# yzang2019/tendermint-fork

Measured on AMD Instinct MI355X. Metric: ed25519 verifies/sec at 1/8 MI355X, higher is better.
Workload: dtype u32 (GF(2^255-19) radix 2^25.5 limbs, int64 accumulate); 1 GPU; C2: raw batch of 1048576 ed25519 signatures per GPU; signatures_per_gpu=1048576, key_cache=False, parallelism=shard-per-gpu x1

## Files before the change

include/tmed25519.h:

```cpp
#ifndef TMED25519_H
#define TMED25519_H

#include <stddef.h>
#include <stdint.h>

#ifdef __cplusplus
extern "C" {
#endif

#define TMED_OK 0
#define TMED_EINVAL (-1)
#define TMED_ENODEV (-2)
#define TMED_EHIP (-3)
#define TMED_ENOMEM (-4)
#define TMED_ENOKEYSET (-5)
#define TMED_EINTERNAL (-6)

typedef struct tmed_ctx tmed_ctx;

int tmed_device_count(void);

int tmed_init(int device, tmed_ctx **out);
void tmed_destroy(tmed_ctx *ctx);
const char *tmed_strerror(int code);
// ... 50 lines not shown
int tmed_verify_batch_keyset_zip215_device(tmed_ctx *ctx, uint64_t handle, const uint32_t *d_val_idx,
                                           const uint8_t *d_sigs, const uint8_t *d_msgs, const uint32_t *d_msg_off,
                                           size_t n, uint8_t *d_out_valid, void *stream);

#define TMED_RULE_GO 0
#define TMED_RULE_ZIP215 1
int tmed_set_rule(tmed_ctx *ctx, int rule);
int tmed_rule(const tmed_ctx *ctx);


typedef struct {
  const char *chain_id;
  uint32_t chain_id_len;
  int64_t height;
  int32_t round;
  const uint8_t *block_hash;
  uint32_t block_hash_len;
  uint32_t psh_total;
  const uint8_t *psh_hash;
  uint32_t psh_hash_len;
} tmed_vote_template;

int tmed_vote_sign_bytes(const tmed_vote_template *t, size_t n, const uint8_t *flags, const int64_t *ts_seconds,
                         const int32_t *ts_nanos, uint8_t *out, size_t out_cap, uint32_t *out_off, size_t *out_len);


int tmed_valu_peak(tmed_ctx *ctx, int kind, double *giga_ops_per_s);

void tmed_test_pool_jitter(int max_us);
void tmed_test_stream_delay(int us);

int tmed_test_joint_rows(tmed_ctx *ctx, const uint8_t *a, const uint8_t *r, const uint8_t *dneg, size_t n,
                         uint8_t *rows);

int tmed_test_b_table_entry(tmed_ctx *ctx, int table, uint32_t window, uint32_t j, int32_t out[30]);
int tmed_test_table_chain(tmed_ctx *ctx, int table, uint64_t handle, int radix_bits, uint32_t corrupt_window,
                          uint32_t corrupt_j, uint64_t *rows, uint64_t *n_bad, uint64_t first_bad[16]);

int tmed_test_zip_msm(tmed_ctx *ctx, uint32_t n, const uint8_t *points, const int16_t *digits, const uint8_t *c,
                      uint32_t lo, uint32_t cnt, int32_t windows[640], uint32_t ctot[8], uint32_t *flag);

int tmed_test_key_order(tmed_ctx *ctx, const uint32_t *val_idx, uint32_t n, uint32_t nkeys, uint32_t index_base,
                        uint32_t *perm_out, uint32_t *cursor_out, uint32_t *nbins_out, uint32_t *shift_out);
int tmed_test_finish(tmed_ctx *ctx, uint32_t m, const int32_t *xyz, const uint8_t *r, const uint32_t *perm,
                     uint32_t fin_base, const uint8_t *bits_in, uint8_t *bits_out);
int tmed_test_finish_zip215(tmed_ctx *ctx, uint32_t m, const int32_t *xyz, const uint8_t *r, const uint32_t *perm,
                            uint32_t fin_base, const uint8_t *bits_in, uint8_t *bits_out);

int tmed_debug_zero_bits(void *out, size_t cap, size_t *n);


typedef struct {
  const uint8_t *hash;
  uint32_t hash_len;
  uint32_t psh_total;
  const uint8_t *psh_hash;
  uint32_t psh_hash_len;
} tmed_block_id;

typedef struct {
  size_t n;
  const uint8_t *pubkeys;
  const int64_t *powers;
  const uint8_t *addresses;
  int64_t total_power;
  uint64_t keyset;
// ... 331 lines not shown
```

tendermint-fork_amd/csrc/kernels.h:

```cpp
#pragma once
#include <hip/hip_runtime.h>
#include <stddef.h>
#include <stdint.h>

#include "ge25519.h"
#include "signbytes.h"

namespace tmed {

struct KernelTimer {
  static constexpr int kMax = 160;
  hipEvent_t ev[kMax];
  int kind[kMax];
  int n = 0;
  void mark(hipStream_t s, int k) {
    if (n < kMax) { kind[n] = k; (void)hipEventRecord(ev[n++], s); }
  }
};

constexpr uint32_t kThreadsPerBlock = 256;
constexpr uint32_t kSlabSlotBytes = 8 * 128;
constexpr uint32_t kSlabJointSlotBytes = 12 * 128;
inline size_t slab_bytes(uint32_t slots) { return (size_t)slots * kSlabJointSlotBytes; }

// ... 63 lines not shown
                             hipStream_t stream);
hipError_t launch_comb_fill(const int32_t *bases, uint32_t n, int4 *comb, hipStream_t stream);
#ifndef TMED_COMBA_BITS
#define TMED_COMBA_BITS 12
#endif
constexpr int kCombABits = TMED_COMBA_BITS;
constexpr int kCombAWindows = 253 / kCombABits;
constexpr int kCombATopField = 253 - kCombABits * (kCombAWindows - 1);
constexpr uint32_t kCombAEntries = (1u << (kCombABits - 1)) + 1;
constexpr uint32_t kCombATopMax = (1u << (kCombATopField - 1)) + 1;
constexpr uint32_t kCombATopGroups = (kCombATopMax + 127) / 128;
constexpr uint32_t kCombATopEntries = kCombATopGroups * 128 + 1;
static_assert(kCombABits >= 10 && kCombABits <= 12 && kCombATopField >= kCombABits, "comb radix");
constexpr size_t kCombARowsPerKey = (size_t)(kCombAWindows - 1) * kCombAEntries + kCombATopEntries;
constexpr size_t kCombABytesPerKey = kCombARowsPerKey * kCombEntryInt4 * 16;
constexpr size_t comba_row(int w, uint32_t j) { return (size_t)w * kCombAEntries + j; }
hipError_t launch_build_comba(const uint8_t *pubs, uint32_t n, int32_t *bases, int4 *comba, hipStream_t stream);
hipError_t launch_verify_keyset(const uint32_t *val_idx, uint32_t nkeys, const uint8_t *key_pub, const uint8_t *key_ok,
                                const int4 *const *acomb, const int4 *bcomb, const uint8_t *sig, const uint8_t *msgs,
                                const uint32_t *off, uint32_t n, uint8_t *out, int4 *prep, uint32_t stride,
                                int4 *fin, int4 *fin_pre, hipStream_t stream, bool msg_slots = false,
                                KernelTimer *timer = nullptr, uint32_t *perm = nullptr,
                                uint32_t *order_scratch = nullptr, const int4 *bcomb24 = nullptr,
                                const int4 *const *acomba = nullptr, int rule = kRuleGo);
constexpr uint32_t kKeyOrderMaxKeys = 1u << 24;
uint32_t key_order_scratch_words(uint32_t n, uint32_t nkeys);
uint32_t key_order_shift(uint32_t nkeys);
hipError_t launch_key_order(const uint32_t *val_idx, uint32_t n, uint32_t nkeys, uint32_t *scratch, uint32_t *perm,
                            uint32_t index_base, hipStream_t stream);

hipError_t launch_test_delay(hipStream_t stream, uint32_t us);
hipError_t launch_test_joint_rows(const uint8_t *a, const uint8_t *r, const uint8_t *dneg, uint32_t n, int4 *rows,
                                  hipStream_t stream);
struct ChainPlan {
  const int4 *base;
  const int4 *const *chunks;
  const uint8_t *ok;
  uint64_t units, rows_per_unit;
  uint32_t windows, entries, top_entries, top_chain_last, step_bits;
};
hipError_t launch_table_chain(const ChainPlan &p, uint64_t *d_out, hipStream_t stream);
hipError_t launch_table_corrupt(int4 *row, hipStream_t stream);
hipError_t launch_window_stats(const int4 *prep, uint32_t stride, uint32_t count, uint32_t *d_hist,
                               hipStream_t stream);

constexpr uint32_t kLatMax = 1u << 16;
struct VoteAsm;
hipError_t launch_verify_keyset_lat(const uint32_t *val_idx, uint32_t nkeys, const uint8_t *key_pub, const uint8_t *key_ok,
                                    const int4 *const *acomb, const int4 *bcomb, const uint8_t *sig, const uint8_t *msgs,
                                    const uint32_t *off, uint32_t n, uint8_t *out, int4 *fin, int4 *dec,
                                    hipStream_t stream, bool msg_slots = false, const VoteAsm *va = nullptr,
                                    int rule = kRuleGo);

constexpr uint32_t kGLatMax = 1u << 16;
constexpr size_t kGLatHandBytes = (size_t)kGLatMax * (6 * 2 + 7) * 16;
struct VoteAsm {
  const uint8_t *tmpl;
  const uint32_t *tmpl_idx;
  const uint8_t *flags;
  const int64_t *ts_sec;
  const int32_t *ts_nanos;
};

hipError_t launch_verify_glat(const uint8_t *pub, const uint8_t *sig, const uint8_t *msgs, const uint32_t *off,
                              uint32_t n, uint8_t *out, const int4 *comb16, int4 *hand, hipStream_t stream,
                              bool msg_slots = false, KernelTimer *timer = nullptr, const VoteAsm *va = nullptr);
// ... 21 lines not shown
```

tendermint-fork_amd/csrc/kernels.hip:

```cpp
#include "kernels.h"
#include "verify_core.h"
#include "verify_hs.h"
#include "kernel_util.h"
#include "rows.h"
#include "votes_dev.h"

namespace tmed {

__device__ int4 kIdentityRow[8] = {{1, 0, 0, 0}, {0, 0, 0, 0}, {1, 0, 0, 0}, {0, 0, 0, 0},
                                          {1, 0, 0, 0}, {0, 0, 0, 0}, {0, 0, 0, 0}, {0, 0, 0, 0}};

__device__ __forceinline__ void slab_st(int4 *p, int4 v) { *p = v; }
__device__ __forceinline__ int4 slab_ld(const int4 *p) { return *p; }

template <int ROWS>
struct SlabTabN {
  int4 *base;
  uint32_t slot;

  __device__ __forceinline__ const int4 *row(int j) const {
    return j == 0 ? kIdentityRow : base + ((size_t)slot * ROWS + (j - 1)) * 8;
  }

  __device__ __forceinline__ void store(int j, const ge_cached &c) const {
    if (j == 0) return;
    int4 *r = base + ((size_t)slot * ROWS + (j - 1)) * 8;
    const fe *fs[4] = {&c.YpX, &c.YmX, &c.Z, &c.T2d};
#pragma unroll
    for (int f = 0; f < 4; f++) {
      uint32_t w[8];
      fe_pack256(w, *fs[f]);
      slab_st(r + 2 * f, make_int4((int)w[0], (int)w[1], (int)w[2], (int)w[3]));
      slab_st(r + 2 * f + 1, make_int4((int)w[4], (int)w[5], (int)w[6], (int)w[7]));
    }
  }
  int4 pv[8];
  __device__ __forceinline__ void prefetch(int j, bool swap = false) {
    const int4 *r = row(j);
    const int sx = swap ? 2 : 0;
#pragma unroll
    for (int q = 0; q < 8; q++) pv[q] = slab_ld(r + (q < 4 ? (q ^ sx) : q));
  }
  __device__ __forceinline__ void take(ge_cached &c) const {
    fe *fs[4] = {&c.YpX, &c.YmX, &c.Z, &c.T2d};
#pragma unroll
    for (int f = 0; f < 4; f++) {
      const uint32_t w[8] = {(uint32_t)pv[2 * f].x, (uint32_t)pv[2 * f].y, (uint32_t)pv[2 * f].z,
                             (uint32_t)pv[2 * f].w, (uint32_t)pv[2 * f + 1].x, (uint32_t)pv[2 * f + 1].y,
                             (uint32_t)pv[2 * f + 1].z, (uint32_t)pv[2 * f + 1].w};
      fe_unpack256(*fs[f], w);
    }
  }
};
using SlabTab = SlabTabN<8>;
using SlabTabJ = SlabTabN<kJointRows>;
static_assert(kSlabSlotBytes == 8 * 128 && kSlabJointSlotBytes == kJointRows * 128, "slab rows are 128 B");

typedef __attribute__((address_space(1))) void global_void;
typedef __attribute__((address_space(3))) void lds_void;

template <int BITS>
struct BPf {
  static constexpr int kBits = BITS;
  const int4 *tab;
  int4 *buf;
  uint32_t lane;
  __device__ __forceinline__ void prefetch(int j) const {
    __builtin_amdgcn_s_waitcnt(0xc07f);
#pragma unroll
    for (int q = 0; q < 8; q++)
      __builtin_amdgcn_global_load_lds((global_void *)(tab + (size_t)j * 8 + q), (lds_void *)(buf + q * 64), 16, 0, 0);
  }
  __device__ __forceinline__ void take(ge_niels &e) const { niels_load(e, buf + lane, 64); }
};

constexpr uint32_t kHsBlock = kThreadsPerBlock;

constexpr int kPrepWaves = 3;
__global__ __launch_bounds__(kHsBlock, kPrepWaves) void verify_prep_kernel(
    const uint8_t *__restrict__ pub, const uint8_t *__restrict__ sig, MsgSrc ms, uint32_t base, uint32_t count,
    int4 *__restrict__ prep, uint32_t stride, uint32_t *__restrict__ place) {
  const uint32_t slot = blockIdx.x * blockDim.x + threadIdx.x;
  if (place && slot == 0) place[0] = place[1] = 0;
  if (slot >= count) return;
  const uint32_t i = base + slot;
  uint32_t pw[8];
  bool sok;
  {
    uint32_t sw[16], k[8], h[16];
// ... 107 lines not shown
  for (int j = 0; j < 8; j++) { w[j] = (int32_t)cr[j]; w[13 + j] = (int32_t)er[j]; }
#pragma unroll
  for (int j = 0; j < 5; j++) w[8 + j] = (int32_t)dr[j];
#pragma unroll
  for (int j = 0; j < 10; j++) { w[21 + j] = Rx.v[j]; w[31 + j] = Ry.v[j]; }
  w[41] = ((ok && rok) ? 1 : 0) | (dneg ? 2 : 0) | (W << 8);
  w[42] = (int32_t)slot;
  w[43] = 0;
#pragma unroll
  for (int q = 4; q < 9; q++) {
    const int4 v = prep[(size_t)q * stride + slot];
    w[28 + 4 * q] = v.x; w[29 + 4 * q] = v.y; w[30 + 4 * q] = v.z; w[31 + 4 * q] = v.w;
  }
  const bool front = W > kHsWSmall;
  const uint64_t act = __ballot(1), sm = __ballot(front);
  const uint32_t lane = threadIdx.x & 63u;
  const uint64_t below = lane ? (~0ull >> (64 - lane)) : 0ull;
  uint32_t fs = 0, fl = 0;
  if (lane == (uint32_t)__builtin_ctzll(act)) {
    const uint32_t ns = (uint32_t)__builtin_popcountll(sm), nl = (uint32_t)__builtin_popcountll(act & ~sm);
    if (ns) fs = atomicAdd(&place[0], ns);
    if (nl) fl = atomicAdd(&place[1], nl);
  }
  const int leader = __builtin_ctzll(act);
  fs = (uint32_t)__shfl((int)fs, leader);
  fl = (uint32_t)__shfl((int)fl, leader);
  const uint32_t pos = front ? fs + (uint32_t)__builtin_popcountll(sm & below)
                             : count - 1u - (fl + (uint32_t)__builtin_popcountll(act & ~sm & below));
#pragma unroll
  for (int q = 0; q < kPrepHsInt4; q++)
    prep2[(size_t)q * stride + pos] = make_int4(w[4 * q], w[4 * q + 1], w[4 * q + 2], w[4 * q + 3]);
}

struct HsDigitsDev {
  const int4 *p2;
  uint32_t stride, slot;
  bool active;
  __device__ __forceinline__ uint32_t word(int w) const {
    return active ? reinterpret_cast<const uint32_t *>(p2 + (size_t)(w >> 2) * stride + slot)[w & 3] : 0x88888888u;
  }
  __device__ __forceinline__ uint32_t cword(int w) const { return word(w); }
  __device__ __forceinline__ uint32_t dword(int w) const { return w < 5 ? word(8 + w) : 0x88888888u; }
};

constexpr int kHsWaves = 2;
template <int BB>
__global__ __launch_bounds__(kHsBlock, kHsWaves) void verify_main_hs_kernel(
    uint32_t base, uint32_t count, const int4 *__restrict__ prep, const int4 *__restrict__ prep2, uint32_t stride,
    int4 *__restrict__ slab, const int4 *__restrict__ btab, uint8_t *__restrict__ out, int zip215) {
  __shared__ int4 sbl[kHsBlock / 64][8 * 64];
  __shared__ int4 sbh[kHsBlock / 64][8 * 64];
  const uint32_t slot = blockIdx.x * blockDim.x + threadIdx.x;
  const bool active = slot < count;
  int32_t w[64];
#pragma unroll
  for (int q = 3; q < kPrepHsInt4; q++) {
    const int4 v = active ? prep2[(size_t)q * stride + slot] : make_int4(0, 0, 0, 0);
    w[4 * q] = v.x; w[4 * q + 1] = v.y; w[4 * q + 2] = v.z; w[4 * q + 3] = v.w;
  }
  uint32_t er[8];
#pragma unroll
  for (int j = 0; j < 8; j++) er[j] = (uint32_t)w[13 + j];
  if (BB == 16) {
    uint32_t e[8];
#pragma unroll
    for (int j = 0; j < 8; j++) e[j] = er[j];
    sc_recode_b<16>(er, e);
  }
  fe Rx, Ry;
#pragma unroll
  for (int j = 0; j < 10; j++) { Rx.v[j] = w[21 + j]; Ry.v[j] = w[31 + j]; }
  ge_p3 A;
#pragma unroll
  for (int j = 0; j < 10; j++) { A.X.v[j] = w[44 + j]; A.Y.v[j] = w[54 + j]; }
  if (!active) { fe_1(A.Y); fe_1(Ry); }
  fe_1(A.Z);
  fe_mul(A.T, A.X, A.Y);
  const int flags = w[41];
  int W = active ? (flags >> 8) : 29;
#pragma unroll
  for (int o = 32; o > 0; o >>= 1) {
    const int x = __shfl_xor(W, o);
    W = x > W ? x : W;
  }
  W = __builtin_amdgcn_readfirstlane(W);
  if (W < 29) W = 29;
  if (W > 64) W = 64;
  const uint32_t lane = threadIdx.x & 63u, wv = threadIdx.x >> 6;
  const HsDigitsDev ds{prep2, stride, slot, active};
  SlabTabJ tj{slab, slot};
  const size_t hi = BB == 26 ? (size_t)kB26Entries * kCombEntryInt4 : (size_t)8 * kB16Entries * kCombEntryInt4;
  BPf<BB> bl{btab, sbl[wv], lane};
  BPf<BB> bh{btab + hi, sbh[wv], lane};
  const bool id = verify_main_hsj(ds, (flags & 2) != 0, er, W, A, Rx, Ry, tj, bl, bh, zip215 != 0);
  if (active) out[base + (uint32_t)w[42]] = ((flags & 1) && id) ? 1 : 0;
}

__global__ __launch_bounds__(kThreadsPerBlock) void window_stats_kernel(const int4 *__restrict__ prep2, uint32_t stride,
                                                                       uint32_t count, uint32_t *__restrict__ lane_hist,
                                                                       uint32_t *__restrict__ wave_hist) {
  __shared__ uint32_t lh[65], wh[65];
  for (uint32_t b = threadIdx.x; b < 65; b += blockDim.x) lh[b] = wh[b] = 0;
  __syncthreads();
  const uint32_t slot = blockIdx.x * blockDim.x + threadIdx.x;
  const bool active = slot < count;
  int W = active ? (prep2[(size_t)10 * stride + slot].y >> 8) : 0;
  if (W < 0 || W > 64) W = 64;
  if (active) atomicAdd(&lh[W], 1u);
  int m = W;
#pragma unroll
  for (int o = 32; o > 0; o >>= 1) {
    const int x = __shfl_xor(m, o);
    m = x > m ? x : m;
  }
  if ((threadIdx.x & 63u) == 0 && slot < count) atomicAdd(&wh[m], 1u);
  __syncthreads();
  for (uint32_t b = threadIdx.x; b < 65; b += blockDim.x) {
    if (lh[b]) atomicAdd(&lane_hist[b], lh[b]);
    if (wh[b]) atomicAdd(&wave_hist[b], wh[b]);
  }
}

__global__ __launch_bounds__(kHsBlock) void test_joint_rows_kernel(const uint8_t *__restrict__ a,
                                                                   const uint8_t *__restrict__ r,
                                                                   const uint8_t *__restrict__ dneg, uint32_t n,
                                                                   int4 *__restrict__ rows) {
  const uint32_t i = blockIdx.x * blockDim.x + threadIdx.x;
  if (i >= n) return;
  uint32_t aw[8], rw[8];
  load_row_words(aw, a + 32 * (size_t)i, 2);
  load_row_words(rw, r + 32 * (size_t)i, 2);
  ge_p3 A, R, P, Q;
  ge_frombytes_go(A, aw);
  ge_frombytes_go(R, rw);
  hs_points(P, Q, dneg[i] != 0, A, R.X, R.Y);
  SlabTabJ tj{rows, i};
  build_table_joint(tj, P, Q);
}

hipError_t launch_test_joint_rows(const uint8_t *a, const uint8_t *r, const uint8_t *dneg, uint32_t n, int4 *rows,
                                  hipStream_t stream) {
  if (n == 0) return hipSuccess;
  hipLaunchKernelGGL(test_joint_rows_kernel, dim3((n + kHsBlock - 1) / kHsBlock), dim3(kHsBlock), 0, stream, a, r,
                     dneg, n, rows);
  return hipGetLastError();
}

__global__ __launch_bounds__(64) void test_delay_kernel(uint32_t iters) {
  for (uint32_t i = 0; i < iters; i++) __builtin_amdgcn_s_sleep(127);
}

hipError_t launch_test_delay(hipStream_t stream, uint32_t us) {
  if (us == 0) return hipSuccess;
  hipLaunchKernelGGL(test_delay_kernel, dim3(1), dim3(64), 0, stream, (us < 100000u ? us : 100000u) / 3u + 1u);
  return hipGetLastError();
}

hipError_t launch_window_stats(const int4 *prep, uint32_t stride, uint32_t count, uint32_t *d_hist,
                               hipStream_t stream) {
  if (count == 0) return hipSuccess;
  hipError_t e = hipMemsetAsync(d_hist, 0, 2 * 65 * sizeof(uint32_t), stream);
  if (e != hipSuccess) return e;
  hipLaunchKernelGGL(window_stats_kernel, dim3((count + kThreadsPerBlock - 1) / kThreadsPerBlock),
                     dim3(kThreadsPerBlock), 0, stream, prep + (size_t)kPrepInt4 * stride, stride, count, d_hist,
                     d_hist + 65);
  return hipGetLastError();
}

struct FinDev {
  const int4 *fin;
  int4 *pre;
  const uint8_t *sig;
  uint8_t *out;
  uint32_t fin_base, lane, L, m;
  const uint32_t *perm;
  __device__ __forceinline__ int count() const { return lane < m ? (int)((m - lane + L - 1) / L) : 0; }
  __device__ __forceinline__ uint32_t slot(int j) const { return lane + (uint32_t)j * L; }
// ... 722 lines not shown
```

tendermint-fork_amd/csrc/tmed_capi.hip:

```cpp
#include <hip/hip_runtime.h>
#include <stdlib.h>
#include <string.h>

#include <algorithm>
#include <map>
#include <mutex>
#include <new>
#include <string>

#include "../../include/tmed25519.h"
#include "kernels.h"

#include "call_frame.h"
#include "median_host.h"

using namespace tmed;

extern "C" {

int tmed_device_count(void) {
  int n = 0;
  if (hipGetDeviceCount(&n) != hipSuccess) return 0;
  return n;
}
// ... 375 lines not shown
    const hipError_t er = scratch_release(c, c->stream);
    if (e == hipSuccess) e = er;
  }
  uint32_t h[130];
  if (e == hipSuccess) e = hipMemcpyAsync(h, d, sizeof h, hipMemcpyDeviceToHost, c->stream);
  const int rc = finish_call(c, c->stream, e);
  (void)hipFree(d);
  if (rc != TMED_OK) return rc;
  for (int w = 0; w < 65; w++) { lane_hist[w] = h[w]; wave_hist[w] = h[65 + w]; }
  return TMED_OK;
}

int tmed_test_joint_rows(tmed_ctx *c, const uint8_t *a, const uint8_t *r, const uint8_t *dneg, size_t n,
                         uint8_t *rows) {
  if (!c || !a || !r || !dneg || !rows || n == 0 || n > 65536) return TMED_EINVAL;
  std::lock_guard<std::mutex> lk(c->mu);
  (void)hipSetDevice(c->device);
  uint8_t *d_in = nullptr;
  int4 *d_rows = nullptr;
  const size_t row_bytes = n * kSlabJointSlotBytes;
  hipError_t e = hipMalloc((void **)&d_in, 65 * n);
  if (e == hipSuccess) e = hipMalloc((void **)&d_rows, row_bytes);
  if (e == hipSuccess) e = hipMemcpyAsync(d_in, a, 32 * n, hipMemcpyHostToDevice, c->stream);
  if (e == hipSuccess) e = hipMemcpyAsync(d_in + 32 * n, r, 32 * n, hipMemcpyHostToDevice, c->stream);
  if (e == hipSuccess) e = hipMemcpyAsync(d_in + 64 * n, dneg, n, hipMemcpyHostToDevice, c->stream);
  if (e == hipSuccess) e = launch_test_joint_rows(d_in, d_in + 32 * n, d_in + 64 * n, (uint32_t)n, d_rows, c->stream);
  if (e == hipSuccess) e = hipMemcpyAsync(rows, d_rows, row_bytes, hipMemcpyDeviceToHost, c->stream);
  const int rc = finish_call(c, c->stream, e);
  if (d_in) (void)hipFree(d_in);
  if (d_rows) (void)hipFree(d_rows);
  return rc;
}

static bool b_table_plan(const tmed_ctx *c, int table, ChainPlan &p) {
  p = ChainPlan{};
  p.units = 1;
  switch (table) {
    case 0: p.base = c->d_bcomb; p.windows = kCombWindows; p.entries = kCombEntries; p.step_bits = 8; break;
    case 1: p.base = c->d_b16; p.windows = 1; p.entries = kB16Entries; p.step_bits = 16; break;
    case 2: p.base = c->d_bcomb16; p.windows = 16; p.entries = kB16Entries; p.step_bits = 16; break;
    case 3: p.base = c->d_b26; p.windows = 2; p.entries = kB26Entries; p.step_bits = 128; break;
    case 4: p.base = c->d_b24; p.windows = kB24Windows; p.entries = kB24Entries; p.step_bits = 24; break;
    default: return false;
  }
  p.top_entries = p.entries;
  p.top_chain_last = table == 4 ? 32767u : p.entries - 1;
  p.rows_per_unit = (uint64_t)p.windows * p.entries;
  return p.base != nullptr;
}

int tmed_test_b_table_entry(tmed_ctx *c, int table, uint32_t window, uint32_t j, int32_t out[30]) {
  if (!c || !out) return TMED_EINVAL;
  std::lock_guard<std::mutex> lk(c->mu);
  ChainPlan p;
  if (!b_table_plan(c, table, p) || window >= p.windows || j >= p.entries) return TMED_EINVAL;
  (void)hipSetDevice(c->device);
  int4 row[kCombEntryInt4];
  if (hipStreamSynchronize(c->stream) != hipSuccess || hipDeviceSynchronize() != hipSuccess) return TMED_EHIP;
  const int4 *src = p.base + ((size_t)window * p.entries + j) * kCombEntryInt4;
  if (hipMemcpy(row, src, sizeof(row), hipMemcpyDeviceToHost) != hipSuccess) return TMED_EHIP;
  const int32_t *w = reinterpret_cast<const int32_t *>(row);
  for (int i = 0; i < 30; i++) out[i] = w[i];
  return TMED_OK;
}

int tmed_test_table_chain(tmed_ctx *c, int table, uint64_t handle, int radix_bits, uint32_t corrupt_window,
// ... 226 lines not shown
```

tendermint-fork_amd/csrc/verify_hs.h:

```cpp
#pragma once
#include <math.h>

#include "verify_core.h"

namespace tmed {

TMED_HD void sc_const_8L(uint32_t n[8]) {
  const uint32_t c[8] = {0xe7ae9f68u, 0xc09318d2u, 0x17bce6b2u, 0xa6f7cef5u, 0u, 0u, 0u, 0x80000000u};
#pragma unroll
  for (int i = 0; i < 8; i++) n[i] = c[i];
}

TMED_HD int bitlen_words(const uint32_t *x, int n) {
  int b = 0;
#pragma unroll
  for (int i = 0; i < n; i++)
    if (x[i]) b = 32 * i + 32 - __builtin_clz(x[i]);
  return b;
}

TMED_HD double words_to_double(const uint32_t *x, int n) {
  double r = 0.0;
#pragma unroll
  for (int i = n - 1; i >= 0; i--) r = r * 4294967296.0 + (double)x[i];
// ... 240 lines not shown
                            HsDigits &dg, uint32_t er[8], bool &dneg, ge_p3 &A, fe &Rx, fe &Ry, int &W,
                            bool raw_e = false) {
  uint32_t k[8], s[8];
  const bool ok = verify_prep(pubw, sigw, msg, mlen, k, s, A);
  int Wl;
  const bool rok = hs_prep_r(k, s, sigw, dg.cr, dg.dr, er, dneg, Rx, Ry, Wl, false, raw_e, &W);
  return ok && rok;
}

TMED_HD void words4_shl16(uint32_t x[4]) {
#pragma unroll
  for (int i = 3; i > 0; i--) x[i] = (x[i] << 16) | (x[i - 1] >> 16);
  x[0] <<= 16;
}

TMED_HD int hs_b26_digit(const uint32_t x[4], int m) {
  const int o = 26 * m, q = o >> 5, r = o & 31;
  const uint64_t lo = x[q], hi = q + 1 < 4 ? x[q + 1] : 0u;
  const uint32_t u = (uint32_t)(((hi << 32) | lo) >> r) & 0x3ffffffu;
  const uint32_t below = m ? (x[(o - 1) >> 5] >> ((o - 1) & 31)) & 1u : 0u;
  return (int)(u + below) - (int)((u >> 25) << 26);
}
TMED_HD void hs_b26_digits(int dl[5], int dh[5], const uint32_t er[8]) {
  const uint32_t el[4] = {er[0], er[1], er[2], er[3]}, eh[4] = {er[4], er[5], er[6], er[7]};
#pragma unroll
  for (int m = 0; m < 5; m++) { dl[m] = hs_b26_digit(el, m); dh[m] = hs_b26_digit(eh, m); }
}

template <class BL, class BH>
TMED_HD void hs_b26_add(ge_p1p1 &t, ge_p3 &r, int m, const int dl[5], const int dh[5], BL &bl, BH &bh) {
  ge_niels nb;
  ge_p1p1_to_p3(r, t);
  bl.take(nb);
  if (m > 0) bl.prefetch(dl[m - 1] < 0 ? -dl[m - 1] : dl[m - 1]);
  niels_apply_sign(nb, dl[m] < 0);
  ge_madd_niels(t, r, nb, false);
  ge_p1p1_to_p3(r, t);
  bh.take(nb);
  if (m > 0) bh.prefetch(dh[m - 1] < 0 ? -dh[m - 1] : dh[m - 1]);
  niels_apply_sign(nb, dh[m] < 0);
  ge_madd_niels(t, r, nb, false);
}

template <class DS, class TA, class TR, class BL, class BH>
TMED_HD void hs_straus(ge_p2 &out, const DS &ds, const uint32_t er[8], int W, TA &ta, TR &tr, BL &bl, BH &bh) {
  constexpr bool b26 = BL::kBits == 26;
  static_assert(BL::kBits == 16 || BL::kBits == 26, "B windows of radix 2^16 or 2^26");
  uint32_t el[4] = {er[0], er[1], er[2], er[3]}, eh[4] = {er[4], er[5], er[6], er[7]};
  int d26l[5] = {0, 0, 0, 0, 0}, d26h[5] = {0, 0, 0, 0, 0};
  if (b26) {
    hs_b26_digits(d26l, d26h, er);
    bl.prefetch(d26l[4] < 0 ? -d26l[4] : d26l[4]);
    bh.prefetch(d26h[4] < 0 ? -d26h[4] : d26h[4]);
  } else {
    const int dl = (int)(el[3] >> 16) - 32768, dh = (int)(eh[3] >> 16) - 32768;
    bl.prefetch(dl < 0 ? -dl : dl);
    bh.prefetch(dh < 0 ? -dh : dh);
  }
  ge_p2 q;
  ge_p1p1 t;
  ge_p3 r;
  ge_cached ca;
  ge_niels nb;
  uint32_t cw = 0, dw = 0;
#pragma unroll 1
  for (int n = W - 1; n >= 0; n--) {
    if (n == W - 1 || (n & 7) == 7) {
      cw = ds.cword(n >> 3);
      dw = ds.dword(n >> 3);
    }
    if (n == W - 1) {
      const int dc = hs_top_digit(cw, W < 64 ? ((W & 7) ? cw : ds.cword(W >> 3)) : 0u, W);
      const int dd = hs_top_digit(dw, W < 64 ? ((W & 7) ? dw : ds.dword(W >> 3)) : 0u, W);
      const int c1 = dc < 8 ? dc : 8, d1 = dd < 8 ? dd : 8;
      ta.prefetch(c1, false);
      ta.take(ca);
      ta.prefetch(dc - c1, false);
      ge_cached_to_p3(r, ca);
      ta.take(ca);
      tr.prefetch(d1, false);
      ge_add_cached_pre(t, r, ca, false);
      ge_p1p1_to_p3(r, t);
      tr.take(ca);
      tr.prefetch(dd - d1, false);
      ge_add_cached_pre(t, r, ca, false);
      ge_p1p1_to_p3(r, t);
// ... 26 lines not shown
      words4_shl16(eh);
      ge_p1p1_to_p3(r, t);
      bl.take(nb);
      const int nl = (int)(el[3] >> 16) - 32768;
      bl.prefetch(nl < 0 ? -nl : nl);
      niels_apply_sign(nb, dl < 0);
      ge_madd_niels(t, r, nb, false);
      ge_p1p1_to_p3(r, t);
      bh.take(nb);
      const int nh = (int)(eh[3] >> 16) - 32768;
      bh.prefetch(nh < 0 ? -nh : nh);
      niels_apply_sign(nb, dh < 0);
      ge_madd_niels(t, r, nb, false);
    }
    ge_p1p1_to_p2(q, t);
  }
  out = q;
}

TMED_HD void hs_split4(int D, int &h, int &l) {
  l = ((D + 2) & 3) - 2;
  h = (D - l) >> 2;
}

template <class DS, class TJ, class BL, class BH>
TMED_HD void hs_straus_joint(ge_p2 &out, const DS &ds, const uint32_t er[8], int W, TJ &tj, BL &bl, BH &bh) {
  constexpr bool b26 = BL::kBits == 26;
  static_assert(BL::kBits == 16 || BL::kBits == 26, "B windows of radix 2^16 or 2^26");
  uint32_t el[4] = {er[0], er[1], er[2], er[3]}, eh[4] = {er[4], er[5], er[6], er[7]};
  int d26l[5] = {0, 0, 0, 0, 0}, d26h[5] = {0, 0, 0, 0, 0};
  if (b26) {
    hs_b26_digits(d26l, d26h, er);
    bl.prefetch(d26l[4] < 0 ? -d26l[4] : d26l[4]);
    bh.prefetch(d26h[4] < 0 ? -d26h[4] : d26h[4]);
  } else {
    const int dl = (int)(el[3] >> 16) - 32768, dh = (int)(eh[3] >> 16) - 32768;
    bl.prefetch(dl < 0 ? -dl : dl);
    bh.prefetch(dh < 0 ? -dh : dh);
  }
  ge_p2 q;
  ge_p1p1 t;
  ge_p3 r;
  ge_cached ca;
  ge_niels nb;
  uint32_t cw = ds.cword((W - 1) >> 3), dw = ds.dword((W - 1) >> 3), cwn = cw, dwn = dw;
  int ih = 0, il;
  {
    const int dc = hs_top_digit(cw, W < 64 ? ((W & 7) ? cw : ds.cword(W >> 3)) : 0u, W);
    const int dd = hs_top_digit(dw, W < 64 ? ((W & 7) ? dw : ds.dword(W >> 3)) : 0u, W);
    int hc, lc, hd, ld;
    hs_split4(dc, hc, lc);
    hs_split4(dd, hd, ld);
    const int c1 = hc < 2 ? hc : 2, d1 = hd < 2 ? hd : 2;
    tj.prefetch(joint_index(c1, d1), false);
    tj.take(ca);
    tj.prefetch(joint_index(hc - c1, hd - d1), false);
    ge_cached_to_p3(r, ca);
    tj.take(ca);
    il = joint_index(lc, ld);
    tj.prefetch(il < 0 ? -il : il, il < 0);
    ge_add_cached_pre(t, r, ca, false);
    ge_p1p1_to_p2(q, t);
  }
#pragma unroll 1
  for (int n = W - 1; n >= 0; n--) {
    if (n > 0 && ((n - 1) & 7) == 7) {
      cwn = ds.cword((n - 1) >> 3);
// ... 110 lines not shown
```

tendermint-fork_amd/tmed/_native.py:

```python
from __future__ import annotations

import ctypes
import os

PKG_ROOT = os.path.dirname(os.path.dirname(os.path.abspath(__file__)))
LIB_PATH = os.environ.get("TMED_LIB") or os.path.join(PKG_ROOT, "lib", "libtmed25519_hip.so")

TMED_OK = 0
TMED_EINVAL = -1
TMED_ENODEV = -2
TMED_EHIP = -3
TMED_ENOMEM = -4
TMED_ENOKEYSET = -5
TMED_EINTERNAL = -6

_lib = None


class TmedError(RuntimeError):
    def __init__(self, code: int, what: str = ""):
        self.code = code
        msg = lib().tmed_strerror(code).decode() if _lib is not None else str(code)
        super().__init__("%s: %s (code %d)" % (what or "tmed", msg, code))

# ... 60 lines not shown
    l.tmed_kernel_times.restype = I
    l.tmed_kernel_times.argtypes = [P, ctypes.POINTER(ctypes.c_float), ctypes.POINTER(ctypes.c_int)]
    l.tmed_last_kernel_ms.restype = ctypes.c_float
    l.tmed_last_kernel_ms.argtypes = [P]
    l.tmed_window_stats.restype = I
    l.tmed_window_stats.argtypes = [P, P, P]
    l.tmed_b_window_bits.restype = I
    l.tmed_b_window_bits.argtypes = [P]
    l.tmed_keyset_b_window_bits.restype = I
    l.tmed_keyset_b_window_bits.argtypes = [P]
    l.tmed_keyset_a_window_bits.restype = I
    l.tmed_keyset_a_window_bits.argtypes = [P, ctypes.c_uint64]
    l.tmed_keyset_comb_entry.restype = I
    l.tmed_keyset_comb_entry.argtypes = [P, ctypes.c_uint64, ctypes.c_uint32, ctypes.c_int, ctypes.c_uint32,
                                         ctypes.c_uint32, P]
    l.tmed_host_alloc.restype = I
    l.tmed_host_alloc.argtypes = [SZ, ctypes.POINTER(ctypes.c_void_p)]
    l.tmed_host_free.restype = I
    l.tmed_host_free.argtypes = [P]
    l.tmed_host_register.restype = I
    l.tmed_host_register.argtypes = [P, SZ]
    l.tmed_host_unregister.restype = I
    l.tmed_host_unregister.argtypes = [P]
    l.tmed_verify_batch_zip215.argtypes = [P, P, P, P, P, P, SZ, P]
    l.tmed_verify_batch_zip215_device.argtypes = [P, P, P, P, P, SZ, P, P]
    l.tmed_zip215_set_seed.argtypes = [P]
    l.tmed_zip215_stats.argtypes = [P]
    l.tmed_test_pool_jitter.restype = None
    l.tmed_test_pool_jitter.argtypes = [I]
    l.tmed_test_stream_delay.restype = None
    l.tmed_test_stream_delay.argtypes = [I]
    l.tmed_test_joint_rows.restype = I
    l.tmed_test_joint_rows.argtypes = [P, P, P, P, SZ, P]
    l.tmed_test_b_table_entry.restype = I
    l.tmed_test_b_table_entry.argtypes = [P, I, ctypes.c_uint32, ctypes.c_uint32, P]
    l.tmed_test_table_chain.restype = I
    l.tmed_test_table_chain.argtypes = [P, I, ctypes.c_uint64, I, ctypes.c_uint32, ctypes.c_uint32,
                                        ctypes.POINTER(ctypes.c_uint64), ctypes.POINTER(ctypes.c_uint64), P]
    l.tmed_test_zip_msm.restype = I
    l.tmed_test_zip_msm.argtypes = [P, ctypes.c_uint32, P, P, P, ctypes.c_uint32, ctypes.c_uint32, P, P,
                                    ctypes.POINTER(ctypes.c_uint32)]
    l.tmed_test_key_order.restype = I
    l.tmed_test_key_order.argtypes = [P, P, ctypes.c_uint32, ctypes.c_uint32, ctypes.c_uint32, P, P,
                                      ctypes.POINTER(ctypes.c_uint32), ctypes.POINTER(ctypes.c_uint32)]
    l.tmed_test_finish.restype = I
    l.tmed_test_finish.argtypes = [P, ctypes.c_uint32, P, P, P, ctypes.c_uint32, P, P]
    l.tmed_test_finish_zip215.restype = I
    l.tmed_test_finish_zip215.argtypes = [P, ctypes.c_uint32, P, P, P, ctypes.c_uint32, P, P]
    l.tmed_debug_zero_bits.restype = I
    l.tmed_debug_zero_bits.argtypes = [P, SZ, ctypes.POINTER(SZ)]
    _lib = l
    return l


EXPORTED_SYMBOLS = [
    "tmed_device_count", "tmed_init", "tmed_destroy", "tmed_strerror",
    "tmed_verify_batch", "tmed_verify_batch_device",
    "tmed_sign_batch", "tmed_sign_batch_device", "tmed_last_kernel_ms",
    "tmed_vote_sign_bytes", "tmed_valu_peak", "tmed_verify_commits", "tmed_verify_commits_with",
    "tmed_test_pool_jitter", "tmed_test_stream_delay", "tmed_test_joint_rows", "tmed_debug_zero_bits",
    "tmed_test_b_table_entry", "tmed_test_table_chain", "tmed_test_zip_msm",
    "tmed_test_key_order", "tmed_test_finish", "tmed_test_finish_zip215",
    "tmed_set_rule", "tmed_rule", "tmed_verify_batch_keyset_zip215", "tmed_verify_batch_keyset_zip215_device",
    "tmed_keyset_load", "tmed_keyset_free", "tmed_keyset_extend", "tmed_verify_batch_keyset",
    "tmed_keycache_config", "tmed_keycache_stats", "tmed_keycache_flush", "tmed_keycache_warm", "tmed_keycache_wait", "tmed_verify_batch_keyset_device",
    "tmed_set_kernel_timing", "tmed_kernel_times", "tmed_blocksync_verify", "tmed_blocksync_submit", "tmed_blocksync_wait",
    "tmed_merkle_roots", "tmed_valset_hashes", "tmed_header_hashes", "tmed_partset_roots",
    "tmed_commit_hashes", "tmed_txs_hashes",
    "tmed_merkle_proofs", "tmed_partset_proofs", "tmed_txs_proofs", "tmed_merkle_proofs_verify",
    "tmed_light_verify", "tmed_light_verify_with",
    "tmed_median_times", "tmed_median_times_host",
    "tmed_verify_votes", "tmed_verify_votes_host", "tmed_votes_sign_bytes", "tmed_votes_last_prepare_ms",
    "tmed_verify_duplicate_votes", "tmed_evidence_kernel_times", "tmed_evidence_hashes", "tmed_evidence_bytes",
    "tmed_verify_duplicate_votes_host",
    "tmed_verify_commits_multi", "tmed_blocksync_verify_multi", "tmed_window_stats", "tmed_b_window_bits", "tmed_keyset_b_window_bits", "tmed_keyset_a_window_bits", "tmed_keyset_comb_entry", "tmed_seam_phase_us",
    "tmed_verify_batch_zip215", "tmed_verify_batch_zip215_device", "tmed_zip215_set_seed", "tmed_zip215_stats",
    "tmed_host_alloc", "tmed_host_free", "tmed_host_register", "tmed_host_unregister",
]
```

Measured before the change: 111.0 million verifies/s.

## Keep two joint-table rows in LDS for the b26 half-size Straus kernel

For the b26 table path, the per-thread joint precomputation table now keeps rows 1 and 5 in LDS (packed, with Z dropped as implicitly one) instead of the global slab, reusing LDS freed by sharing a single B prefetch buffer between the low and high B tables. Digit and prep loads use a wave-uniform base plus lane index, and later prep fields are loaded only after the table is built, to cut register pressure. The B-table prefetch order is also reordered so the low and high lookups share one buffer. It adds LDS usage per block, which may lower occupancy, and adds a test hook for the LDS rows.

```diff
diff --git a/include/tmed25519.h b/include/tmed25519.h
--- a/include/tmed25519.h
+++ b/include/tmed25519.h
@@ -106,6 +106,9 @@
 
 int tmed_test_joint_rows(tmed_ctx *ctx, const uint8_t *a, const uint8_t *r, const uint8_t *dneg, size_t n,
                          uint8_t *rows);
+
+int tmed_test_lds_rows(tmed_ctx *ctx, const uint8_t *a, const uint8_t *r, const uint8_t *dneg, size_t n,
+                       uint8_t *rows, int32_t *out);
 
 int tmed_test_b_table_entry(tmed_ctx *ctx, int table, uint32_t window, uint32_t j, int32_t out[30]);
 int tmed_test_table_chain(tmed_ctx *ctx, int table, uint64_t handle, int radix_bits, uint32_t corrupt_window,
diff --git a/tendermint-fork_amd/csrc/kernels.h b/tendermint-fork_amd/csrc/kernels.h
--- a/tendermint-fork_amd/csrc/kernels.h
+++ b/tendermint-fork_amd/csrc/kernels.h
@@ -119,6 +119,8 @@
 hipError_t launch_test_delay(hipStream_t stream, uint32_t us);
 hipError_t launch_test_joint_rows(const uint8_t *a, const uint8_t *r, const uint8_t *dneg, uint32_t n, int4 *rows,
                                   hipStream_t stream);
+hipError_t launch_test_lds_rows(const uint8_t *a, const uint8_t *r, const uint8_t *dneg, uint32_t n, int4 *rows,
+                                int32_t *out, hipStream_t stream);
 struct ChainPlan {
   const int4 *base;
   const int4 *const *chunks;
diff --git a/tendermint-fork_amd/csrc/kernels.hip b/tendermint-fork_amd/csrc/kernels.hip
--- a/tendermint-fork_amd/csrc/kernels.hip
+++ b/tendermint-fork_amd/csrc/kernels.hip
@@ -55,6 +55,79 @@
 using SlabTab = SlabTabN<8>;
 using SlabTabJ = SlabTabN<kJointRows>;
 static_assert(kSlabSlotBytes == 8 * 128 && kSlabJointSlotBytes == kJointRows * 128, "slab rows are 128 B");
+
+constexpr int kLdsRowInt4 = 6;
+constexpr uint32_t kLdsRowsInt4 = 2 * kLdsRowInt4 * kThreadsPerBlock;
+typedef int v4i __attribute__((ext_vector_type(4)));
+typedef __attribute__((address_space(1))) v4i glb_v4i;
+typedef __attribute__((address_space(3))) v4i lds_v4i;
+struct SlabLdsTabJ {
+  int4 *blk;
+  uint32_t tid;
+  int4 *lds;
+  __device__ __forceinline__ int4 *slab_row(int j) const { return blk + (tid * kJointRows + (uint32_t)(j - 1)) * 8u; }
+
+  __device__ __forceinline__ static bool in_lds(int j) { return j == 1 || j == 5; }
+
+  __device__ __forceinline__ void store(int j, const ge_cached &c) const {
+    if (j == 0) return;
+    if (in_lds(j)) {
+      lds_v4i *r = (lds_v4i *)lds + (j == 5 ? kLdsRowInt4 : 0) * kThreadsPerBlock;
+      const fe *fs[3] = {&c.YpX, &c.YmX, &c.T2d};
+#pragma unroll
+      for (int f = 0; f < 3; f++) {
+        uint32_t w[8];
+        fe_pack256(w, *fs[f]);
+        r[(2 * f) * kThreadsPerBlock] = v4i{(int)w[0], (int)w[1], (int)w[2], (int)w[3]};
+        r[(2 * f + 1) * kThreadsPerBlock] = v4i{(int)w[4], (int)w[5], (int)w[6], (int)w[7]};
+      }
+      return;
+    }
+    glb_v4i *r = (glb_v4i *)slab_row(j);
+    const fe *fs[4] = {&c.YpX, &c.YmX, &c.Z, &c.T2d};
+#pragma unroll
+    for (int f = 0; f < 4; f++) {
+      uint32_t w[8];
+      fe_pack256(w, *fs[f]);
+      r[2 * f] = v4i{(int)w[0], (int)w[1], (int)w[2], (int)w[3]};
+      r[2 * f + 1] = v4i{(int)w[4], (int)w[5], (int)w[6], (int)w[7]};
+    }
+  }
+  v4i pv[8];
+  bool inl, isp, swp;
+  __device__ __forceinline__ void prefetch(int j, bool swap = false) {
+    inl = in_lds(j);
+    isp = j == 5;
+    swp = swap;
+    const glb_v4i *r = (const glb_v4i *)(j == 0 || inl ? kIdentityRow : slab_row(j));
+    const int sx = swap ? 2 : 0;
+#pragma unroll
+    for (int q = 0; q < 8; q++) pv[q] = r[q < 4 ? (q ^ sx) : q];
+  }
+  __device__ __forceinline__ void take(ge_cached &c) {
+    if (inl) {
+      const lds_v4i *r = (const lds_v4i *)lds + (isp ? kLdsRowInt4 : 0) * (int)kThreadsPerBlock;
+      const int sx = swp ? 2 * (int)kThreadsPerBlock : 0;
+      const lds_v4i *a = r + sx, *b = r + (2 * (int)kThreadsPerBlock - sx);
+      pv[0] = a[0];
+      pv[1] = a[kThreadsPerBlock];
+      pv[2] = b[0];
+      pv[3] = b[kThreadsPerBlock];
+      pv[4] = v4i{1, 0, 0, 0};
+      pv[5] = v4i{0, 0, 0, 0};
+      pv[6] = r[4 * kThreadsPerBlock];
+      pv[7] = r[5 * kThreadsPerBlock];
+    }
+    fe *fs[4] = {&c.YpX, &c.YmX, &c.Z, &c.T2d};
+#pragma unroll
+    for (int f = 0; f < 4; f++) {
+      const uint32_t w[8] = {(uint32_t)pv[2 * f].x, (uint32_t)pv[2 * f].y, (uint32_t)pv[2 * f].z,
+                             (uint32_t)pv[2 * f].w, (uint32_t)pv[2 * f + 1].x, (uint32_t)pv[2 * f + 1].y,
+                             (uint32_t)pv[2 * f + 1].z, (uint32_t)pv[2 * f + 1].w};
+      fe_unpack256(*fs[f], w);
+    }
+  }
+};
 
 typedef __attribute__((address_space(1))) void global_void;
 typedef __attribute__((address_space(3))) void lds_void;
@@ -228,39 +301,58 @@
     prep2[(size_t)q * stride + pos] = make_int4(w[4 * q], w[4 * q + 1], w[4 * q + 2], w[4 * q + 3]);
 }
 
+__device__ __forceinline__ uint32_t lane_fresh() {
+  uint32_t z = 0;
+  asm volatile("" : "+v"(z));
+  return __builtin_amdgcn_mbcnt_hi(~0u, __builtin_amdgcn_mbcnt_lo(~0u, z));
+}
+
 struct HsDigitsDev {
   const int4 *p2;
-  uint32_t stride, slot;
+  uint32_t stride, slot0;
   bool active;
   __device__ __forceinline__ uint32_t word(int w) const {
-    return active ? reinterpret_cast<const uint32_t *>(p2 + (size_t)(w >> 2) * stride + slot)[w & 3] : 0x88888888u;
+    const uint32_t u = ((uint32_t)(w >> 2) * stride + slot0) * 4u + (uint32_t)(w & 3);
+    return active ? reinterpret_cast<const uint32_t *>(p2)[u + lane_fresh() * 4u] : 0x88888888u;
   }
   __device__ __forceinline__ uint32_t cword(int w) const { return word(w); }
   __device__ __forceinline__ uint32_t dword(int w) const { return w < 5 ? word(8 + w) : 0x88888888u; }
 };
 
 constexpr int kHsWaves = 2;
+static_assert(kHsBlock == kThreadsPerBlock, "SlabLdsTabJ's lane stride");
+template <int BB>
+struct HsLds;
+template <>
+struct HsLds<26> {
+  int4 bl[kHsBlock / 64][8 * 64];
+  int4 pq[kLdsRowsInt4];
+  __device__ __forceinline__ int4 *bh(uint32_t wv) { return bl[wv]; }
+};
+template <>
+struct HsLds<16> {
+  int4 bl[kHsBlock / 64][8 * 64];
+  int4 bhs[kHsBlock / 64][8 * 64];
+  __device__ __forceinline__ int4 *bh(uint32_t wv) { return bhs[wv]; }
+};
 template <int BB>
 __global__ __launch_bounds__(kHsBlock, kHsWaves) void verify_main_hs_kernel(
     uint32_t base, uint32_t count, const int4 *__restrict__ prep, const int4 *__restrict__ prep2, uint32_t stride,
     int4 *__restrict__ slab, const int4 *__restrict__ btab, uint8_t *__restrict__ out, int zip215) {
-  __shared__ int4 sbl[kHsBlock / 64][8 * 64];
-  __shared__ int4 sbh[kHsBlock / 64][8 * 64];
+  __shared__ HsLds<BB> sm;
   const uint32_t slot = blockIdx.x * blockDim.x + threadIdx.x;
   const bool active = slot < count;
   int32_t w[64];
 #pragma unroll
-  for (int q = 3; q < kPrepHsInt4; q++) {
+  for (int q = BB == 26 ? 5 : 3; q < kPrepHsInt4; q++) {
     const int4 v = active ? prep2[(size_t)q * stride + slot] : make_int4(0, 0, 0, 0);
     w[4 * q] = v.x; w[4 * q + 1] = v.y; w[4 * q + 2] = v.z; w[4 * q + 3] = v.w;
   }
   uint32_t er[8];
-#pragma unroll
-  for (int j = 0; j < 8; j++) er[j] = (uint32_t)w[13 + j];
-  if (BB == 16) {
+  if constexpr (BB == 16) {
     uint32_t e[8];
 #pragma unroll
-    for (int j = 0; j < 8; j++) e[j] = er[j];
+    for (int j = 0; j < 8; j++) e[j] = (uint32_t)w[13 + j];
     sc_recode_b<16>(er, e);
   }
   fe Rx, Ry;
@@ -283,13 +375,36 @@
   if (W < 29) W = 29;
   if (W > 64) W = 64;
   const uint32_t lane = threadIdx.x & 63u, wv = threadIdx.x >> 6;
-  const HsDigitsDev ds{prep2, stride, slot, active};
-  SlabTabJ tj{slab, slot};
+  const uint32_t slot0 = blockIdx.x * blockDim.x + ((uint32_t)__builtin_amdgcn_readfirstlane((int)threadIdx.x) & ~63u);
+  const HsDigitsDev ds{prep2, stride, slot0, active};
   const size_t hi = BB == 26 ? (size_t)kB26Entries * kCombEntryInt4 : (size_t)8 * kB16Entries * kCombEntryInt4;
-  BPf<BB> bl{btab, sbl[wv], lane};
-  BPf<BB> bh{btab + hi, sbh[wv], lane};
-  const bool id = verify_main_hsj(ds, (flags & 2) != 0, er, W, A, Rx, Ry, tj, bl, bh, zip215 != 0);
-  if (active) out[base + (uint32_t)w[42]] = ((flags & 1) && id) ? 1 : 0;
+  BPf<BB> bl{btab, sm.bl[wv], lane};
+  BPf<BB> bh{btab + hi, sm.bh(wv), lane};
+  bool id;
+  if constexpr (BB == 26) {
+    SlabLdsTabJ tj{slab + (size_t)blockIdx.x * blockDim.x * (kJointRows * 8), threadIdx.x, sm.pq + threadIdx.x};
+    ge_p3 P, Q;
+    hs_points(P, Q, (flags & 2) != 0, A, Rx, Ry);
+    build_table_joint(tj, P, Q);
+#pragma unroll
+    for (int q = 3; q < 6; q++) {
+      const int4 v = active ? prep2[(size_t)q * stride + slot0 + lane_fresh()] : make_int4(0, 0, 0, 0);
+      w[4 * q] = v.x; w[4 * q + 1] = v.y; w[4 * q + 2] = v.z; w[4 * q + 3] = v.w;
+    }
+#pragma unroll
+    for (int j = 0; j < 8; j++) er[j] = (uint32_t)w[13 + j];
+    ge_p2 q;
+    hs_straus_joint(q, ds, er, W, tj, bl, bh);
+    if (zip215) p2_mul8(q);
+    id = p2_is_identity(q);
+  } else {
+    SlabTabJ tj{slab, slot};
+    id = verify_main_hsj(ds, (flags & 2) != 0, er, W, A, Rx, Ry, tj, bl, bh, zip215 != 0);
+  }
+  if (active) {
+    const int4 v = prep2[(size_t)10 * stride + slot0 + lane_fresh()];
+    out[base + (uint32_t)v.z] = ((v.y & 1) && id) ? 1 : 0;
+  }
 }
 
 __global__ __launch_bounds__(kThreadsPerBlock) void window_stats_kernel(const int4 *__restrict__ prep2, uint32_t stride,
@@ -339,6 +454,50 @@
   if (n == 0) return hipSuccess;
   hipLaunchKernelGGL(test_joint_rows_kernel, dim3((n + kHsBlock - 1) / kHsBlock), dim3(kHsBlock), 0, stream, a, r,
                      dneg, n, rows);
+  return hipGetLastError();
+}
+
+__global__ __launch_bounds__(kHsBlock) void test_lds_rows_kernel(const uint8_t *__restrict__ a,
+                                                                 const uint8_t *__restrict__ r,
+                                                                 const uint8_t *__restrict__ dneg, uint32_t n,
+                                                                 int4 *__restrict__ rows, int32_t *__restrict__ out) {
+  __shared__ int4 pq[kLdsRowsInt4];
+  const uint32_t i = blockIdx.x * blockDim.x + threadIdx.x;
+  if (i >= n) return;
+  uint32_t aw[8], rw[8];
+  load_row_words(aw, a + 32 * (size_t)i, 2);
+  load_row_words(rw, r + 32 * (size_t)i, 2);
+  ge_p3 A, R, P, Q;
+  ge_frombytes_go(A, aw);
+  ge_frombytes_go(R, rw);
+  hs_points(P, Q, dneg[i] != 0, A, R.X, R.Y);
+  SlabLdsTabJ tj{rows + (size_t)blockIdx.x * blockDim.x * (kJointRows * 8), threadIdx.x, pq + threadIdx.x};
+  build_table_joint(tj, P, Q);
+  int32_t *o = out + (size_t)i * (kJointRows + 1) * 2 * 40;
+#pragma unroll 1
+  for (int j = 0; j <= kJointRows; j++) {
+#pragma unroll 1
+    for (int s = 0; s < 2; s++) {
+      ge_cached c;
+      tj.prefetch(j, s != 0);
+      tj.take(c);
+#pragma unroll
+      for (int l = 0; l < 10; l++) {
+        o[l] = c.YpX.v[l];
+        o[10 + l] = c.YmX.v[l];
+        o[20 + l] = c.Z.v[l];
+        o[30 + l] = c.T2d.v[l];
+      }
+      o += 40;
+    }
+  }
+}
+
+hipError_t launch_test_lds_rows(const uint8_t *a, const uint8_t *r, const uint8_t *dneg, uint32_t n, int4 *rows,
+                                int32_t *out, hipStream_t stream) {
+  if (n == 0) return hipSuccess;
+  hipLaunchKernelGGL(test_lds_rows_kernel, dim3((n + kHsBlock - 1) / kHsBlock), dim3(kHsBlock), 0, stream, a, r, dneg,
+                     n, rows, out);
   return hipGetLastError();
 }
 
diff --git a/tendermint-fork_amd/csrc/tmed_capi.hip b/tendermint-fork_amd/csrc/tmed_capi.hip
--- a/tendermint-fork_amd/csrc/tmed_capi.hip
+++ b/tendermint-fork_amd/csrc/tmed_capi.hip
@@ -431,6 +431,33 @@
   return rc;
 }
 
+int tmed_test_lds_rows(tmed_ctx *c, const uint8_t *a, const uint8_t *r, const uint8_t *dneg, size_t n, uint8_t *rows,
+                       int32_t *out) {
+  if (!c || !a || !r || !dneg || !rows || !out || n == 0 || n > 65536) return TMED_EINVAL;
+  std::lock_guard<std::mutex> lk(c->mu);
+  (void)hipSetDevice(c->device);
+  uint8_t *d_in = nullptr;
+  int4 *d_rows = nullptr;
+  int32_t *d_out = nullptr;
+  const size_t row_bytes = n * kSlabJointSlotBytes, out_bytes = n * 26 * 40 * sizeof(int32_t);
+  hipError_t e = hipMalloc((void **)&d_in, 65 * n);
+  if (e == hipSuccess) e = hipMalloc((void **)&d_rows, row_bytes);
+  if (e == hipSuccess) e = hipMalloc((void **)&d_out, out_bytes);
+  if (e == hipSuccess) e = hipMemcpyAsync(d_in, a, 32 * n, hipMemcpyHostToDevice, c->stream);
+  if (e == hipSuccess) e = hipMemcpyAsync(d_in + 32 * n, r, 32 * n, hipMemcpyHostToDevice, c->stream);
+  if (e == hipSuccess) e = hipMemcpyAsync(d_in + 64 * n, dneg, n, hipMemcpyHostToDevice, c->stream);
+  if (e == hipSuccess) e = hipMemcpyAsync(d_rows, rows, row_bytes, hipMemcpyHostToDevice, c->stream);
+  if (e == hipSuccess)
+    e = launch_test_lds_rows(d_in, d_in + 32 * n, d_in + 64 * n, (uint32_t)n, d_rows, d_out, c->stream);
+  if (e == hipSuccess) e = hipMemcpyAsync(rows, d_rows, row_bytes, hipMemcpyDeviceToHost, c->stream);
+  if (e == hipSuccess) e = hipMemcpyAsync(out, d_out, out_bytes, hipMemcpyDeviceToHost, c->stream);
+  const int rc = finish_call(c, c->stream, e);
+  if (d_in) (void)hipFree(d_in);
+  if (d_rows) (void)hipFree(d_rows);
+  if (d_out) (void)hipFree(d_out);
+  return rc;
+}
+
 static bool b_table_plan(const tmed_ctx *c, int table, ChainPlan &p) {
   p = ChainPlan{};
   p.units = 1;
diff --git a/tendermint-fork_amd/csrc/verify_hs.h b/tendermint-fork_amd/csrc/verify_hs.h
--- a/tendermint-fork_amd/csrc/verify_hs.h
+++ b/tendermint-fork_amd/csrc/verify_hs.h
@@ -296,12 +296,12 @@
   ge_niels nb;
   ge_p1p1_to_p3(r, t);
   bl.take(nb);
-  if (m > 0) bl.prefetch(dl[m - 1] < 0 ? -dl[m - 1] : dl[m - 1]);
+  bh.prefetch(dh[m] < 0 ? -dh[m] : dh[m]);
   niels_apply_sign(nb, dl[m] < 0);
   ge_madd_niels(t, r, nb, false);
   ge_p1p1_to_p3(r, t);
   bh.take(nb);
-  if (m > 0) bh.prefetch(dh[m - 1] < 0 ? -dh[m - 1] : dh[m - 1]);
+  if (m > 0) bl.prefetch(dl[m - 1] < 0 ? -dl[m - 1] : dl[m - 1]);
   niels_apply_sign(nb, dh[m] < 0);
   ge_madd_niels(t, r, nb, false);
 }
@@ -315,7 +315,6 @@
   if (b26) {
     hs_b26_digits(d26l, d26h, er);
     bl.prefetch(d26l[4] < 0 ? -d26l[4] : d26l[4]);
-    bh.prefetch(d26h[4] < 0 ? -d26h[4] : d26h[4]);
   } else {
     const int dl = (int)(el[3] >> 16) - 32768, dh = (int)(eh[3] >> 16) - 32768;
     bl.prefetch(dl < 0 ? -dl : dl);
@@ -408,7 +407,6 @@
   if (b26) {
     hs_b26_digits(d26l, d26h, er);
     bl.prefetch(d26l[4] < 0 ? -d26l[4] : d26l[4]);
-    bh.prefetch(d26h[4] < 0 ? -d26h[4] : d26h[4]);
   } else {
     const int dl = (int)(el[3] >> 16) - 32768, dh = (int)(eh[3] >> 16) - 32768;
     bl.prefetch(dl < 0 ? -dl : dl);
diff --git a/tendermint-fork_amd/tmed/_native.py b/tendermint-fork_amd/tmed/_native.py
--- a/tendermint-fork_amd/tmed/_native.py
+++ b/tendermint-fork_amd/tmed/_native.py
@@ -116,6 +116,9 @@
     l.tmed_test_stream_delay.argtypes = [I]
     l.tmed_test_joint_rows.restype = I
     l.tmed_test_joint_rows.argtypes = [P, P, P, P, SZ, P]
+    if hasattr(l, "tmed_test_lds_rows"):
+        l.tmed_test_lds_rows.restype = I
+        l.tmed_test_lds_rows.argtypes = [P, P, P, P, SZ, P, P]
     l.tmed_test_b_table_entry.restype = I
     l.tmed_test_b_table_entry.argtypes = [P, I, ctypes.c_uint32, ctypes.c_uint32, P]
     l.tmed_test_table_chain.restype = I
@@ -142,7 +145,7 @@
     "tmed_verify_batch", "tmed_verify_batch_device",
     "tmed_sign_batch", "tmed_sign_batch_device", "tmed_last_kernel_ms",
     "tmed_vote_sign_bytes", "tmed_valu_peak", "tmed_verify_commits", "tmed_verify_commits_with",
-    "tmed_test_pool_jitter", "tmed_test_stream_delay", "tmed_test_joint_rows", "tmed_debug_zero_bits",
+    "tmed_test_pool_jitter", "tmed_test_stream_delay", "tmed_test_joint_rows", "tmed_test_lds_rows", "tmed_debug_zero_bits",
     "tmed_test_b_table_entry", "tmed_test_table_chain", "tmed_test_zip_msm",
     "tmed_test_key_order", "tmed_test_finish", "tmed_test_finish_zip215",
     "tmed_set_rule", "tmed_rule", "tmed_verify_batch_keyset_zip215", "tmed_verify_batch_keyset_zip215_device",
```

New measurement: 114.9 million verifies/s (median of 6 runs). 1.04x the previous value.
